# OnurBasci/Real_Time_Path_Tracing_With_SpatioTemporal_Filtering

Measured on AMD Instinct MI355X. Metric: Mray/s (closest-hit queries / whole-frame time: G-buffer + gradient + trace + a-trous), higher is better.
Workload: dtype f32

## Files before the change

include/rtpt.h:

```cpp
#ifndef RTPT_H
#define RTPT_H

#include <stddef.h>
#include <stdint.h>

#ifdef __cplusplus
extern "C" {
#endif

#define RTPT_ABI_VERSION 5

#define RTPT_OK 0
#define RTPT_E_INVALID (-1)
#define RTPT_E_NOMEM (-2)
#define RTPT_E_DEVICE (-3)
#define RTPT_E_NO_SCENE (-4)
#define RTPT_E_NO_GPU (-5)


typedef struct rtpt_push_constants {
  uint32_t sample_batch;
  uint32_t frameNumber;
  uint32_t _pad0[2];
  float cameraPos[3];
// ... 161 lines not shown
struct rtpt_scene_build_info {
  uint32_t builder, fallback;
  uint32_t n_primitives;
  uint32_t n_nodes, depth;
  uint32_t leaf_pairs;
  float build_ms;
  float upload_ms;
};
int rtpt_scene_build_info(rtpt_ctx* ctx, struct rtpt_scene_build_info* out);
int rtpt_scene_rebuild(rtpt_ctx* ctx);

int rtpt_scene_set_instances(rtpt_ctx* ctx, const float* instance_xforms, uint32_t n_instances);

int rtpt_debug_upload_info(rtpt_ctx* ctx, uint64_t out[4]);

int rtpt_debug_live_device_bytes(uint64_t* out);

int rtpt_debug_reuse_info(rtpt_ctx* ctx, uint64_t out[4]);

int rtpt_debug_reproj_info(rtpt_ctx* ctx, uint64_t out[4]);

int rtpt_debug_defer_info(rtpt_ctx* ctx, uint64_t out[4]);


int rtpt_gbuffer(rtpt_ctx* ctx, const rtpt_ubo* ubo, uint32_t y0, uint32_t y1);
int rtpt_temporal_gradient(rtpt_ctx* ctx, const rtpt_push_constants* pc, uint32_t y0, uint32_t y1);
int rtpt_raytrace(rtpt_ctx* ctx, const rtpt_push_constants* pc, uint32_t y0, uint32_t y1);
int rtpt_temporal_filter(rtpt_ctx* ctx, const rtpt_push_constants* pc, const rtpt_ubo* ubo,
                         uint32_t y0, uint32_t y1);
int rtpt_end_frame(rtpt_ctx* ctx);

int rtpt_present(rtpt_ctx* ctx, void* dst_device, uint32_t y0, uint32_t y1);
int rtpt_present_target(rtpt_ctx* ctx, void* dst_device, uint32_t y0, uint32_t y1);

int rtpt_modulate(rtpt_ctx* ctx, uint32_t y0, uint32_t y1);

int rtpt_sync(rtpt_ctx* ctx);
int rtpt_readback(rtpt_ctx* ctx, rtpt_plane which, void* dst, size_t bytes);
int rtpt_set_plane(rtpt_ctx* ctx, rtpt_plane which, const void* src, size_t bytes);
int rtpt_reset_counters(rtpt_ctx* ctx);
int rtpt_set_count_rows(rtpt_ctx* ctx, uint32_t y0, uint32_t y1);
#define RTPT_DEBUG_HIT_ID 0x1u
#define RTPT_DEBUG_PREV_PIXEL 0x2u
int rtpt_enable_debug(rtpt_ctx* ctx, uint32_t mask);

typedef enum rtpt_kernel_id {
// ... 66 lines not shown
```

real_time_path_tracing_with_spatiotemporal_filtering_amd/abi.py:

```python
from __future__ import annotations

import ctypes as C
import os

import numpy as np

PKG_DIR = os.path.dirname(os.path.abspath(__file__))
REPO_DIR = os.path.dirname(PKG_DIR)
LIB_PATH = os.environ.get("RTPT_LIB_PATH") or os.path.join(PKG_DIR, "librtpt_hip.so")
HEADER_PATH = os.path.join(REPO_DIR, "include", "rtpt.h")

RTPT_OK, RTPT_E_INVALID, RTPT_E_NOMEM, RTPT_E_DEVICE, RTPT_E_NO_SCENE, RTPT_E_NO_GPU = 0, -1, -2, -3, -4, -5
FLAG_EXACT_FILTER, FLAG_FORCE_BVH, FLAG_DIRECT_FILTER, FLAG_NO_PATH_COMPACTION = 0x1, 0x2, 0x4, 0x8
FLAG_EXT_ADAPTIVE_ALPHA, FLAG_EXT_GAUSS5, FLAG_EXT_POW2_STRIDE, FLAG_EXT_DISOCCLUSION = 0x10, 0x20, 0x40, 0x80
FLAG_EXT_VARIANCE = 0x100
FLAG_SINGLE_LAUNCH_PATHS = 0x200
FLAG_NO_FILTER_FUSION = 0x400
FLAG_EXT_SVGF_VARIANCE = 0x800
FLAG_EXT_MASK = 0x9F0
FLAG_DEVICE_BVH_BUILD = 0x1000
FLAG_DEVICE_BVH_SAH = 0x2000
FLAG_EXT_DEMODULATE = 0x8000
FLAG_DEVICE_FLATTEN = 0x4000
BVH_BUILDER_HOST_SAH, BVH_BUILDER_DEVICE_LBVH = 0, 1
# ... 80 lines not shown
        ("max_segments", C.c_uint32), ("samples_per_pixel", C.c_uint32),
        ("sigma_n", C.c_int32), ("sigma_z", C.c_float), ("sigma_l", C.c_float), ("alpha", C.c_float),
        ("light_radius", C.c_float), ("light_intensity", C.c_float), ("first_hit_light_divisor", C.c_float),
        ("fov_slope", C.c_float), ("pixel_jitter", C.c_float), ("ray_offset", C.c_float), ("ray_tmax", C.c_float),
        ("flags", C.c_uint32), ("device", C.c_int32),
    ]


assert C.sizeof(PushConstants) == 112 and C.sizeof(Ubo) == 384 and C.sizeof(SceneBuildInfo) == 32

SYMBOLS = [
    "rtpt_config_default", "rtpt_create", "rtpt_destroy", "rtpt_resize", "rtpt_last_error", "rtpt_set_stream", "rtpt_bind_plane",
    "rtpt_plane_ptr", "rtpt_plane_bytes", "rtpt_set_external_history", "rtpt_stream_wait", "rtpt_scene_upload", "rtpt_gbuffer", "rtpt_temporal_gradient",
    "rtpt_raytrace", "rtpt_temporal_filter", "rtpt_end_frame", "rtpt_sync", "rtpt_readback", "rtpt_set_plane",
    "rtpt_reset_counters", "rtpt_set_count_rows", "rtpt_enable_debug", "rtpt_timing_enable", "rtpt_timing_collect", "rtpt_kernel_name",
    "rtpt_selftest_math", "rtpt_selftest_exhaustive", "rtpt_selftest_div", "rtpt_selftest_trace", "rtpt_util_look_at", "rtpt_util_perspective", "rtpt_util_load_obj", "rtpt_util_bvh_check", "rtpt_util_bvh_check_pairs",
    "rtpt_scene_set_materials", "rtpt_util_load_obj_materials", "rtpt_util_bvh_refit_check", "rtpt_set_external_guides",
    "rtpt_present", "rtpt_debug_bvh_check", "rtpt_present_target", "rtpt_scene_build_info", "rtpt_scene_rebuild",
    "rtpt_debug_reuse_info", "rtpt_debug_bvh_topology", "rtpt_scene_set_instances", "rtpt_debug_upload_info",
    "rtpt_debug_live_device_bytes", "rtpt_modulate", "rtpt_debug_reproj_info", "rtpt_debug_defer_info",
    "rtpt_scene_set_textures", "rtpt_selftest_texture", "rtpt_util_load_obj_texcoords", "rtpt_util_load_obj_map_kd",
    "rtpt_selftest_texture_lod", "rtpt_selftest_texture_footprint", "rtpt_util_texture_chain", "rtpt_selftest_contract",
    "rtpt_scene_set_materials_ext", "rtpt_util_load_obj_materials_ext", "rtpt_selftest_bounce",
    "rtpt_util_load_obj_materials_ni", "rtpt_selftest_refract",
]

CONTRACT_WORDS = ((6, 1), (6, 3), (3, 1), (3, 3), (2, 1), (1, 1), (2, 2), (4, 1), (1, 3), (1, 2), (1, 1), (1, 1), (19, 4), (2, 1),
                  (3, 2), (9, 1), (12, 3), (13, 3), (12, 3), (36, 2), (10, 1), (3, 3), (3, 6))

_lib = None


def load() -> C.CDLL:
    global _lib
    if _lib is not None:
        return _lib
    if not os.path.exists(LIB_PATH):
        raise RtptLibraryMissing(
            f"{LIB_PATH} not found: build it with `python -c 'import __graft_entry__ as g; g.build()'` "
            "(hipcc --offload-arch=gfx950).  There is no CPU fallback for the hot path.")
    lib = C.CDLL(LIB_PATH)
    vp, u32, sz = C.c_void_p, C.c_uint32, C.c_size_t
    lib.rtpt_last_error.restype = C.c_char_p
    lib.rtpt_last_error.argtypes = [vp]
    lib.rtpt_kernel_name.restype = C.c_char_p
    lib.rtpt_kernel_name.argtypes = [C.c_int]
    sigs = {
# ... 22 lines not shown
        "rtpt_set_plane": [vp, C.c_int, vp, sz],
        "rtpt_reset_counters": [vp],
        "rtpt_enable_debug": [vp, u32],
        "rtpt_set_count_rows": [vp, u32, u32],
        "rtpt_timing_enable": [vp, C.c_int],
        "rtpt_timing_collect": [vp, C.POINTER(C.c_double * K_COUNT), C.POINTER(u32 * K_COUNT)],
        "rtpt_selftest_math": [vp, C.c_int, vp, vp, sz],
        "rtpt_selftest_exhaustive": [vp, C.c_int, vp, vp],
        "rtpt_selftest_div": [vp, C.c_int, C.c_uint32, C.c_uint32, vp, vp],
        "rtpt_selftest_trace": [vp, vp, sz, vp, vp],
        "rtpt_selftest_contract": [vp, C.c_int, vp, vp, sz],
        "rtpt_util_load_obj": [C.c_char_p, vp, C.POINTER(u32), vp, C.POINTER(u32)],
        "rtpt_util_bvh_check": [vp, u32, C.POINTER(C.c_uint64 * 8)],
        "rtpt_util_bvh_check_pairs": [vp, u32, C.c_int, C.POINTER(C.c_uint64 * 8)],
        "rtpt_scene_set_materials": [vp, vp, u32, vp, u32],
        "rtpt_util_bvh_refit_check": [vp, vp, u32, C.POINTER(C.c_uint64 * 8)],
        "rtpt_debug_bvh_check": [vp, C.POINTER(C.c_uint64 * 8)],
        "rtpt_scene_build_info": [vp, C.POINTER(SceneBuildInfo)],
        "rtpt_scene_rebuild": [vp],
        "rtpt_debug_bvh_topology": [vp, vp, C.POINTER(u32), vp, C.POINTER(u32)],
        "rtpt_debug_reuse_info": [vp, C.POINTER(C.c_uint64 * 4)],
        "rtpt_debug_reproj_info": [vp, C.POINTER(C.c_uint64 * 4)],
        "rtpt_debug_defer_info": [vp, C.POINTER(C.c_uint64 * 4)],
        "rtpt_scene_set_instances": [vp, vp, u32],
        "rtpt_debug_upload_info": [vp, C.POINTER(C.c_uint64 * 4)],
        "rtpt_debug_live_device_bytes": [C.POINTER(C.c_uint64)],
        "rtpt_util_load_obj_materials": [C.c_char_p, vp, C.POINTER(u32), vp, C.POINTER(u32)],
        "rtpt_scene_set_textures": [vp, vp, vp, u32, vp, u32, vp, sz],
        "rtpt_selftest_texture": [vp, u32, vp, sz, vp],
        "rtpt_util_load_obj_texcoords": [C.c_char_p, vp, C.POINTER(u32)],
        "rtpt_util_load_obj_map_kd": [C.c_char_p, vp, C.POINTER(sz), C.POINTER(u32)],
        "rtpt_selftest_texture_lod": [vp, u32, vp, vp, sz, vp],
        "rtpt_selftest_texture_footprint": [vp, vp, sz, u32, vp, vp],
        "rtpt_util_texture_chain": [u32, u32, C.POINTER(u32), C.POINTER(C.c_uint64)],
        "rtpt_scene_set_materials_ext": [vp, vp, u32, vp, u32],
        "rtpt_util_load_obj_materials_ext": [C.c_char_p, vp, C.POINTER(u32), vp, C.POINTER(u32)],
        "rtpt_selftest_bounce": [vp, vp, vp, sz],
        "rtpt_util_load_obj_materials_ni": [C.c_char_p, vp, C.POINTER(u32), vp, C.POINTER(u32)],
        "rtpt_selftest_refract": [vp, vp, vp, sz],
    }
    for name, args in sigs.items():
        fn = getattr(lib, name)
        fn.restype = C.c_int
        fn.argtypes = args
    lib.rtpt_util_look_at.restype = None
    lib.rtpt_util_look_at.argtypes = [vp, vp, vp, vp]
# ... 198 lines not shown
    def scene_build_info(self) -> dict:
        info = SceneBuildInfo()
        _check(self._lib.rtpt_scene_build_info(self._h, C.byref(info)))
        return {name: getattr(info, name) for name, _ in SceneBuildInfo._fields_}

    def scene_rebuild(self):
        _check(self._lib.rtpt_scene_rebuild(self._h))

    def reuse_info(self) -> dict:
        out = (C.c_uint64 * 4)()
        _check(self._lib.rtpt_debug_reuse_info(self._h, C.byref(out)))
        return dict(zip(("frames_skipped", "reproj_stores", "reproj_loads", "tags_invalidated"), (int(v) for v in out)))

    def reproj_info(self) -> dict:
        out = (C.c_uint64 * 4)()
        _check(self._lib.rtpt_debug_reproj_info(self._h, C.byref(out)))
        return dict(zip(("stores", "loads", "invalidations", "plane_bytes"), (int(v) for v in out)))

    def defer_info(self) -> dict:
        out = (C.c_uint64 * 4)()
        _check(self._lib.rtpt_debug_defer_info(self._h, C.byref(out)))
        return dict(zip(("recorded", "launched_in_trace", "launched_alone", "spare_bytes"), (int(v) for v in out)))

    def set_materials(self, tri_material: np.ndarray | None, materials: np.ndarray | None):
        if tri_material is None or materials is None:
            _check(self._lib.rtpt_scene_set_materials(self._h, None, 0, None, 0))
            return
        tri = np.ascontiguousarray(tri_material, np.uint32)
        mats = np.ascontiguousarray(materials, np.float32).reshape(-1, 6)
        _check(self._lib.rtpt_scene_set_materials(self._h, _ptr(tri), len(tri), _ptr(mats), len(mats)))

    def set_textures(self, tri_uv=None, tri_texture=None, textures=None, texels=None):
        if tri_uv is None or tri_texture is None or textures is None or texels is None:
            _check(self._lib.rtpt_scene_set_textures(self._h, None, None, 0, None, 0, None, 0))
            return
        uv = np.ascontiguousarray(tri_uv, np.float32).reshape(-1, 6)
        tri = np.ascontiguousarray(tri_texture, np.uint32).ravel()
        if len(uv) != len(tri):
            raise ValueError("one uv record and one texture index per triangle")
        desc = np.ascontiguousarray(textures, np.uint32).reshape(-1, 4)
        tex = np.ascontiguousarray(texels, np.float32).reshape(-1, 4)
        _check(self._lib.rtpt_scene_set_textures(self._h, _ptr(uv), _ptr(tri), len(tri), _ptr(desc), len(desc), _ptr(tex), len(tex)))

    def gbuffer(self, ubo: Ubo, y0=0, y1=0):
        _check(self._lib.rtpt_gbuffer(self._h, C.byref(ubo), y0, y1))

# ... 167 lines not shown
```

real_time_path_tracing_with_spatiotemporal_filtering_amd/csrc/api_context.hip:

```cpp
#include "api_internal.hpp"

#include <atomic>

namespace rtpt_impl {

thread_local std::string g_err;

int fail(int code, const std::string& msg) {
  g_err = msg;
  return code;
}


size_t frame_blocks(const rtpt_ctx* c) {
  const size_t tiles = ((static_cast<size_t>(c->cfg.width) + 63) / 64) * ((static_cast<size_t>(c->cfg.row_end - c->cfg.row_begin) + 3) / 4);
  return std::max(tiles, static_cast<size_t>(c->n_cu > 0 ? c->n_cu : 256) * 8);
}
int ensure_stack_spill(rtpt_ctx* c, size_t blocks) {
  if (!c->scene.use_bvh) return RTPT_OK;
  const size_t depth = static_cast<size_t>(c->scene.tree.bvh_depth + 2 < 8 ? 8 : c->scene.tree.bvh_depth + 2);
  const size_t lds = std::min<size_t>(depth, static_cast<size_t>(c->bvh_stack_lds));
  if (depth <= lds || blocks <= c->stack_spill_blocks) return RTPT_OK;
  if (c->stack_spill.ptr) {
    hipError_t e = hipStreamSynchronize(c->stream);
// ... 329 lines not shown
  if (const char* v = std::getenv("RTPT_LBVH_ORDER")) c->lbvh_by_height = !std::strcmp(v, "height");
  if (const char* v = std::getenv("RTPT_NO_TRACE_FUSION")) c->fuse_trace = std::atoi(v) == 0;
  if (const char* v = std::getenv("RTPT_NO_FRAME_REUSE")) c->frame_reuse = std::atoi(v) == 0;
  if (const char* v = std::getenv("RTPT_NO_REPROJ_REUSE")) c->reproj_reuse = std::atoi(v) == 0;
  if (const char* v = std::getenv("RTPT_TRACE_POOL")) c->trace_pool = std::atoi(v) != 0;
  if (const char* v = std::getenv("RTPT_TEX_BOUNCE_SPREAD")) {
    const float f = std::strtof(v, nullptr);
    if (f > 0.0f && f <= 64.0f) c->tex_bounce_spread = f;
  }
  if (const char* v = std::getenv("RTPT_PT_WINDOW")) c->trace_window = static_cast<uint32_t>(std::max(0, std::atoi(v)));
  if (const char* v = std::getenv("RTPT_CHAIN_G1")) c->filter_policy.chain_g_pin = std::atoi(v);
  if (const char* v = std::getenv("RTPT_CHAIN_GENERIC")) c->filter_policy.chain_generic = std::atoi(v);
  if (const char* v = std::getenv("RTPT_CHAIN_WG_PER_CU")) c->filter_policy.chain_wg_per_cu = std::atoi(v);
  if (const char* v = std::getenv("RTPT_CHAIN_SKEW")) {
    c->filter_policy.chain_skew = c->filter_policy.chain_skew2 = std::atoi(v);
    if (const char* comma = std::strchr(v, ',')) c->filter_policy.chain_skew2 = std::atoi(comma + 1);
  }
  if (const char* v = std::getenv("RTPT_CHAIN_BW")) c->filter_policy.chain_bw = std::atoi(v);
  if (const char* v = std::getenv("RTPT_NO_FINAL_DEFER")) c->final_defer = std::atoi(v) == 0;
  if (const char* v = std::getenv("RTPT_FINAL_FRONT")) {
    c->filter_policy.final_front = std::atoi(v);
    if (const char* comma = std::strchr(v, ',')) c->filter_policy.final_front_share = std::atoi(comma + 1);
  }
  if (const char* v = std::getenv("RTPT_CHAIN_SW")) c->filter_policy.chain_sw = std::atoi(v);
  if (const char* v = std::getenv("RTPT_CHAIN_SW_G1")) c->filter_policy.chain_sw_g1 = std::atoi(v);
  if (const char* v = std::getenv("RTPT_CHAIN_SW_G3")) c->filter_policy.chain_sw_g3 = std::atoi(v);
  if (const char* v = std::getenv("RTPT_CHAIN_MAX")) c->chain_max = std::max(1, std::min(3, std::atoi(v)));
  if (const char* v = std::getenv("RTPT_CHAIN_FINAL")) c->chain_final = std::atoi(v) != 0;
  if (const char* v = std::getenv("RTPT_BVH_STACK_LDS")) c->bvh_stack_lds = std::max(1, std::atoi(v));
  if (const char* v = std::getenv("RTPT_CHAIN_MIN_PIXELS")) c->chain_min_pixels = std::atoll(v);
  int rc = alloc_planes(c);
  if (rc != RTPT_OK) {
    rtpt_destroy(c);
    return rc;
  }
  *out = c;
  return RTPT_OK;
}

int rtpt_destroy(rtpt_ctx* c) {
  if (!c) return RTPT_OK;
  (void)hipSetDevice(c->device);
  (void)final_flush(c);
  if (c->own_stream) (void)hipStreamSynchronize(c->own_stream);
  for (auto& t : c->timed) {
    (void)hipEventDestroy(t.start);
// ... 145 lines not shown
  }
  if (mask != c->debug_mask) reuse_invalidate(c, nullptr);
  c->debug_mask = mask;
  return RTPT_OK;
}

int rtpt_debug_reuse_info(rtpt_ctx* c, uint64_t out[4]) {
  if (!c || !out) return fail(RTPT_E_INVALID, "NULL argument");
  for (int i = 0; i < 4; i++) out[i] = c->reuse_info[i];
  return RTPT_OK;
}

int rtpt_debug_reproj_info(rtpt_ctx* c, uint64_t out[4]) {
  if (!c || !out) return fail(RTPT_E_INVALID, "NULL argument");
  for (int i = 0; i < 3; i++) out[i] = c->reproj_info[i];
  out[3] = c->reproj.bytes;
  return RTPT_OK;
}

int rtpt_debug_defer_info(rtpt_ctx* c, uint64_t out[4]) {
  if (!c || !out) return fail(RTPT_E_INVALID, "NULL argument");
  for (int i = 0; i < 3; i++) out[i] = c->defer_info[i];
  out[3] = c->color[3].bytes;
  return RTPT_OK;
}

int rtpt_debug_live_device_bytes(uint64_t* out) {
  if (!out) return fail(RTPT_E_INVALID, "NULL argument");
  *out = g_live_device_bytes.load();
  return RTPT_OK;
}

int rtpt_debug_upload_info(rtpt_ctx* c, uint64_t out[4]) {
  if (!c || !out) return fail(RTPT_E_INVALID, "NULL argument");
  for (int i = 0; i < 4; i++) out[i] = c->upload_info[i];
  return RTPT_OK;
}

int rtpt_sync(rtpt_ctx* c) {
  if (!c) return fail(RTPT_E_INVALID, "ctx is NULL");
  HIP_TRY(hipSetDevice(c->device));
  FLUSH_FILTER(c);
  HIP_TRY(hipStreamSynchronize(c->stream));
  return RTPT_OK;
}

// ... 113 lines not shown
```

real_time_path_tracing_with_spatiotemporal_filtering_amd/csrc/api_internal.hpp:

```cpp
#pragma once
#include <hip/hip_runtime.h>

#include <algorithm>
#include <cmath>
#include <cstdio>
#include <cstdlib>
#include <cfloat>
#include <cstring>
#include <new>
#include <string>
#include <vector>

#include "../../include/rtpt.h"
#include "bvh.hpp"
#include "kernels.hpp"
#include "rtpt_math.hpp"


namespace rtpt_impl {


extern thread_local std::string g_err;
int fail(int code, const std::string& msg);

// ... 203 lines not shown
  rt::GbufferArgs pending_gb{};
  bool pending_gb_valid = false;
  bool fuse_trace = true;
  bool frame_reuse = true;
  uint64_t scene_gen = 0;
  K1Key pending_key;
  PlaneTag<K0Key> tag_vis[2], tag_worldpos, tag_depth, tag_normals;
  PlaneTag<K1Key> tag_gradient;
  uint64_t reuse_info[4] = {0, 0, 0, 0};
  bool reproj_reuse = true;
  Buf reproj;
  PlaneTag<ReprojKey> tag_reproj;
  PlaneTag<ReprojKey> reproj_last;
  uint64_t reproj_info[4] = {0, 0, 0, 0};
  bool trace_pool = false;
  uint32_t trace_window = 0;
  float tex_bounce_spread = rt::kTexBounceSpread;
  Buf path_pool;
  rt::FilterPolicy filter_policy;
  bool final_defer = true;
  bool deferred_valid = false;
  DeferredFinal deferred;
  uint64_t defer_info[4] = {0, 0, 0, 0};
  std::vector<FilterCall> pending;
  int chain_max = 2;
  bool chain_final = false;
  int64_t chain_min_pixels = 1000000;

  int bvh_stack_lds = 16;
  Buf stack_spill;
  size_t stack_spill_blocks = 0;

  int timing_period = 0;
  uint64_t frames_ended = 0;
  bool timing_now() const { return timing_period > 0 && (frames_ended % static_cast<uint64_t>(timing_period)) == 0; }
  std::vector<TimedLaunch> timed;
  std::vector<hipEvent_t> event_pool;

  uint32_t rows() const { return cfg.row_end - cfg.row_begin; }
  Rows stored_rows() const { return Rows(cfg.row_begin, cfg.row_end); }
  bool width_fits_i16() const { return cfg.width < 30000 && cfg.height < 30000; }
  size_t pixels() const { return static_cast<size_t>(rows()) * cfg.width; }
};

namespace rtpt_impl {

// ... 64 lines not shown
```

real_time_path_tracing_with_spatiotemporal_filtering_amd/csrc/api_passes.hip:

```cpp
#include "api_internal.hpp"

namespace rtpt_impl {
void reuse_invalidate(rtpt_ctx* c, const Buf* b) {
  auto kill = [&](auto& tag, const Buf* of) {
    if ((!b || b == of) && tag.valid) {
      tag.valid = false;
      c->reuse_info[3]++;
    }
  };
  kill(c->tag_vis[0], &c->vis[0]);
  kill(c->tag_vis[1], &c->vis[1]);
  kill(c->tag_worldpos, &c->worldpos);
  kill(c->tag_depth, &c->depth);
  kill(c->tag_normals, &c->normals);
  kill(c->tag_gradient, &c->gradient);
  const bool lut = b == &c->scene.lut[0] || b == &c->scene.lut[1];
  if (lut) kill(c->tag_gradient, b);
  if (!b || lut || b == &c->worldpos || b == &c->vis[0] || b == &c->vis[1]) {
    if (c->tag_reproj.valid) c->reproj_info[2]++;
    c->tag_reproj.valid = false;
    c->reproj_last.valid = false;
  }
}
}
// ... 367 lines not shown
  if (take) {
    FrameState& fr = c->frame;
    if (!c->color[fr.color_spare].ptr) {
      if ((rc = alloc_buf(c->color[fr.color_spare], c->pixels() * 16))) return rc;
      HIP_TRY(hipMemsetAsync(c->color[fr.color_spare].ptr, 0, c->pixels() * 16, c->stream));
    }
    std::swap(fr.color_of_role[ROLE_IMAGE], fr.color_spare);
  }
  a.image = static_cast<float4*>(c->color[c->frame.color_of_role[ROLE_IMAGE]].ptr);
  c->frame.alpha_depth[c->frame.color_of_role[ROLE_IMAGE]] = true;
  if ((rc = ensure_stack_spill(c, std::max<size_t>(frame_blocks(c), rt::pathtrace_grid_blocks(a, fused ? &c->pending_gb : nullptr))))) return rc;
  a.scene = scene_view(c);
  if (joined) {
    c->pending_gb.scene = a.scene;
    c->pending_gb_valid = false;
    if (reused)
      c->reuse_info[0]++;
    else
      tag_outputs(c, c->pending_gb, &c->pending_key);
  }
  {
    Timer tm(c, joined ? RTPT_K_GBUFFER_PATHTRACE : RTPT_K_PATHTRACE);
    rt::launch_pathtrace(a, fused ? &c->pending_gb : nullptr, tex_view(c), c->scene.materials_specular, c->stream,
                         take ? &c->deferred.args : nullptr, &c->filter_policy);
  }
  if (take) {
    c->deferred_valid = false;
    c->defer_info[1]++;
  }
  return launch_check(fused ? "gbuffer + temporal_gradient + raytrace" : "raytrace");
}

}

namespace {

bool is_final(int k, int max_it) { return k == max_it && (k & 1); }

struct Reach {
  int stride;
  int64_t reach;
};
Reach filter_reach(uint32_t ext, int k) {
  const int stride = (ext & rt::kExtPow2Stride) ? (1 << (k - 1)) : k;
  return {stride, static_cast<int64_t>(stride) * ((ext & rt::kExtGauss5) ? 2 : 1)};
}
Rows rows_read(const rtpt_ctx* c, uint32_t y0, uint32_t y1, int64_t reach) {
// ... 413 lines not shown
```

real_time_path_tracing_with_spatiotemporal_filtering_amd/csrc/final_split.hpp:

```cpp
#pragma once
#include <cstdint>

#if defined(__HIPCC__)
#define RTPT_FS_HD __host__ __device__
#else
#define RTPT_FS_HD
#endif

namespace rt {

struct FinalSplit {
  uint32_t n_front, n_tail;
  uint32_t front_items, items;
  uint32_t tiles_x, n_tiles;
};

enum : uint32_t { kFinalRoleTile = 0, kFinalRoleFront = 1, kFinalRoleTail = 2 };
struct FinalRole {
  uint32_t role;
  uint32_t index;
};

RTPT_FS_HD inline FinalRole final_role(const FinalSplit& sp, uint32_t block) {
  const uint32_t t = block - sp.n_front;
  if (t < sp.n_tiles) return FinalRole{kFinalRoleTile, t};
  if (block < sp.n_front) return FinalRole{kFinalRoleFront, block};
  return FinalRole{kFinalRoleTail, t - sp.n_tiles};
}
RTPT_FS_HD inline uint32_t final_grid(const FinalSplit& sp) { return sp.n_front + sp.n_tiles + sp.n_tail; }

constexpr uint32_t kFinalWholeListItems = 32;
inline FinalSplit final_split_plan(uint32_t items, uint32_t tiles_x, uint32_t tiles_y, uint32_t n_cu, uint32_t per_cu, int front, int share) {
  const uint32_t cu8 = (n_cu + 7u) / 8u;
  auto clamp = [](int v, uint32_t hi) { return v < 0 ? 0u : (static_cast<uint32_t>(v) > hi ? hi : static_cast<uint32_t>(v)); };
  const uint32_t front_max = cu8 * (per_cu - 1u);
  uint32_t front_slots = front <= 0 ? 0u : (static_cast<uint32_t>(front) < per_cu ? cu8 * static_cast<uint32_t>(front) : static_cast<uint32_t>(front) / 8u);
  front_slots = front_slots < front_max ? front_slots : front_max;
  FinalSplit sp;
  sp.tiles_x = tiles_x;
  sp.n_tiles = tiles_x * tiles_y;
  sp.items = items;
  if (share < 0) share = items >= kFinalWholeListItems * 8u * front_slots ? 100 : 75;
  sp.front_items = front_slots ? static_cast<uint32_t>(static_cast<uint64_t>(items) * clamp(share, 100u) / 100u) : 0u;
  auto group = [](uint32_t n_items, uint32_t slots_per_xcd) {
    const uint32_t per_xcd = (n_items + 7u) / 8u;
    return n_items ? 8u * (per_xcd < slots_per_xcd ? per_xcd : slots_per_xcd) : 0u;
  };
  sp.n_front = group(sp.front_items, front_slots);
  sp.n_tail = group(items - sp.front_items, cu8 * per_cu - front_slots);
  return sp;
}

}
```

real_time_path_tracing_with_spatiotemporal_filtering_amd/csrc/kernels.hip:

```cpp
#include <cstdlib>

#include "atrous_comb.hpp"
#include "final_split.hpp"
#include "pathtrace_tile.hpp"
#include "select.hpp"

namespace rt {
namespace {

__global__ void k_scene_prepare(ScenePrepArgs a) {
  uint32_t i = blockIdx.x * blockDim.x + threadIdx.x;
  if (i >= a.n_tris) return;
  {
    const float* t = a.tris + 9 * static_cast<size_t>(i);
    f3 v0 = ld3(t), v1 = ld3(t + 3), v2 = ld3(t + 6);
    f3 e1 = v1 - v0, e2 = v2 - v0;
    f3 nn = exact::cross(e1, e2);
    a.isect_id[3 * i] = make_float4(v0.x, v0.y, v0.z, e1.x);
    a.isect_id[3 * i + 1] = make_float4(e1.y, e1.z, e2.x, e2.y);
    a.isect_id[3 * i + 2] = make_float4(e2.z, nn.x, nn.y, nn.z);
    f3 n = exact::normalize(nn);
    a.shade[3 * i] = make_float4(v0.x, v0.y, v0.z, n.x);
    a.shade[3 * i + 1] = make_float4(v1.x, v1.y, v1.z, n.y);
    a.shade[3 * i + 2] = make_float4(v2.x, v2.y, v2.z, n.z);
// ... 97 lines not shown
}

template <int BVH, bool DEMOD, int TEX, int SPEC>
__global__ __launch_bounds__(kPtThreads)
__attribute__((amdgpu_waves_per_eu(kPtBvhWaves, kPtBvhWaves)))
void k_gbuffer_pathtrace(PathtraceArgs a, GbufferArgs g, TexView tex) {
  gbuffer_pathtrace_body<BVH, DEMOD, TEX, SPEC>(a, g, tex);
}
template <bool DEMOD, int TEX, int SPEC>
__global__ __launch_bounds__(kPtThreads)
__attribute__((amdgpu_waves_per_eu(kPtWaves, kPtWaves)))
void k_gbuffer_pathtrace_small(PathtraceArgs a, GbufferArgs g, TexView tex) {
  gbuffer_pathtrace_body<0, DEMOD, TEX, SPEC>(a, g, tex);
}

template <int CW>
__global__ __launch_bounds__(kPtThreads)
__attribute__((amdgpu_waves_per_eu(kPtWaves, kPtWaves)))
void k_pathtrace_final(PathtraceArgs a, TexView tex, AtrousArgs f, FinalSplit sp) {
  static_assert(kPtThreads == kShThreads && kPtRows == kShWaves, "the two bodies share the workgroup shape");
  const FinalRole r = final_role(sp, blockIdx.x);
  if (r.role == kFinalRoleTile) {
    pathtrace_tile<0, true, false, false, 0, 0, 1>(a, tex, r.index, sp.tiles_x, a.tiles_y);
  } else {
    extern __shared__ __attribute__((aligned(16))) unsigned char final_lds[];
    const bool front = r.role == kFinalRoleFront;
#if RTPT_TILE_TIMELINE
    FilterTimelineScope tl_(r.role, front ? r.index : sp.n_front + r.index);
#endif
    comb_items<CW, true, false, false, 1, false, false, true, true>(f, final_lds, r.index, front ? sp.n_front : sp.n_tail,
                                                                       front ? 0u : sp.front_items, front ? sp.front_items : sp.items);
  }
}

template <int BVH, int TEX, int SPEC>
__global__ __launch_bounds__(kPtThreads) void k_pathtrace_queue(PathtraceArgs a, TexView tex) {
  extern __shared__ __attribute__((aligned(16))) uint32_t stack[];
  PathState& st = *reinterpret_cast<PathState*>(stack);
  __shared__ uint32_t wave_cnt[kPtRows];
  __shared__ uint32_t q_base;
  __shared__ unsigned int block_rays;
  const int tid = threadIdx.y * kBlockX + threadIdx.x;
  const int wave = __builtin_amdgcn_readfirstlane(static_cast<int>(threadIdx.y));
  const uint32_t lane = threadIdx.x;
  if (tid == 0) block_rays = 0;
  const f3 light_c = ld3(a.light_c);
// ... 112 lines not shown
bool pathtrace_uses_pool(const PathtraceArgs& a) {
  return a.pool_slab && a.scene.use_bvh && a.scene.leaf_pairs && a.compact && a.spp == 1;
}
size_t pathtrace_pool_bytes(int W, int rows) {
  return static_cast<size_t>((W + kBlockX - 1) / kBlockX) * ((rows + kPoolRows - 1) / kPoolRows) * (7u * kPoolPaths * sizeof(float4));
}
#else
constexpr int kPoolRows = kPtRows;
bool pathtrace_uses_pool(const PathtraceArgs&) { return false; }
size_t pathtrace_pool_bytes(int, int) { return 0; }
#endif
bool pathtrace_takes_final(const PathtraceArgs& a, const TexView& tex, int specular) {
  return !a.scene.use_bvh && a.compact && a.spp == 1 && !a.albedo && !tex.records && !specular && !pathtrace_uses_pool(a) && a.g.y1 > a.g.y0;
}
uint32_t pathtrace_grid_blocks(const PathtraceArgs& a, const GbufferArgs* gb) {
  const uint32_t gx = (a.g.W + kBlockX - 1) / kBlockX;
  const int tr = pathtrace_uses_pool(a) ? kPoolRows : kPtRows;
  return gx * ((a.g.y1 - a.g.y0 + tr - 1) / tr + (gb ? (gb->g.y1 - gb->g.y0 + kBlockY - 1) / kBlockY : 0));
}
static FinalSplit final_split(const PathtraceArgs& a, const AtrousArgs& f, const FilterPolicy& pol, uint32_t tiles_x, uint32_t tiles_y) {
  const uint32_t n_cu = a.n_cu > 0 ? static_cast<uint32_t>(a.n_cu) : 256u;
  const uint32_t per_cu = static_cast<uint32_t>(kPtWaves * 4 / kShWaves);
  const uint32_t items = static_cast<uint32_t>(f.tiles_x) * static_cast<uint32_t>(f.tiles_y) * static_cast<uint32_t>(f.stride);
  return final_split_plan(items, tiles_x, tiles_y, n_cu, per_cu, pol.final_front, pol.final_front_share);
}
void launch_pathtrace(const PathtraceArgs& a, const GbufferArgs* gb, const TexView& tex, int specular, hipStream_t s, const AtrousArgs* fin,
                      const FilterPolicy* pol) {
  if (a.g.y1 <= a.g.y0) return;
  dim3 block(kBlockX, kPtRows);
  const bool pool = pathtrace_uses_pool(a);
  const int tile_rows = pool ? kPoolRows : kPtRows;
  const uint32_t tiles_y = (a.g.y1 - a.g.y0 + tile_rows - 1) / tile_rows;
  const dim3 grid((a.g.W + kBlockX - 1) / kBlockX, tiles_y + (gb ? (gb->g.y1 - gb->g.y0 + kBlockY - 1) / kBlockY : 0), 1);
  const size_t stack_bytes = a.scene.use_bvh ? static_cast<size_t>(a.scene.stack_lds) * kPtThreads * 4 : 0;
  size_t dyn = stack_bytes > sizeof(PathState) ? stack_bytes : sizeof(PathState);
  if (fin) {
    if (gb || !pol || !fin->reproj_in || !pathtrace_takes_final(a, tex, specular)) std::abort();
    dyn = dyn > final_role_lds(*fin) ? dyn : final_role_lds(*fin);
  }
  PathtraceArgs b = a;
  b.tiles_y = tiles_y;
  b.multi_off = static_cast<uint32_t>(dyn / 4);
  const size_t dyn_queue = dyn;
  if (a.spp > 1) dyn += 4 * kPtThreads * 4;
  const uint32_t phase0 = a.first_window ? a.first_window : pt_first_window(a.scene.use_bvh != 0);
  const bool split = a.spp == 1 && a.compact && a.queue[0] && a.queue_count && a.max_segments > phase0 &&
                     (a.max_segments <= 2 * phase0 || a.queue[1]);
  b.seg_begin = 0;
  b.seg_end = split ? phase0 : a.max_segments;
  b.q_in = nullptr;
  b.q_in_count = nullptr;
  b.q_out = split ? a.queue[0] : nullptr;
  b.q_out_count = split ? a.queue_count : nullptr;
  if (split) (void)hipMemsetAsync(a.queue_count, 0, 2 * kPathQueues * sizeof(uint32_t), s);
  if (fin) {
    const FinalSplit sp = final_split(a, *fin, *pol, grid.x, tiles_y);
    const dim3 grid1(final_grid(sp));
    hipLaunchKernelGGL(k_pathtrace_final<kFinalRoleCw>, grid1, block, dyn, s, b, tex, *fin, sp);
  } else
#if RTPT_AB_VARIANTS
  if (pool) {
    if (gb)
      hipLaunchKernelGGL((k_pathtrace_pool<true>), grid, block, dyn, s, b, *gb);
    else
      hipLaunchKernelGGL((k_pathtrace_pool<false>), grid, block, dyn, s, b, GbufferArgs{});
  } else
#endif
  with_mode3(scene_mode(a.scene), [&](auto mode) {
    constexpr int M = decltype(mode)::value;
    with_bool(a.albedo != nullptr, [&](auto demod) {
      constexpr bool D = decltype(demod)::value;
      with_mode3(tex_mode(tex), [&](auto tmode) {
        constexpr int T = decltype(tmode)::value;
        with_mode3(spec_mode(specular), [&](auto spec) {
          constexpr int S = decltype(spec)::value;
          if (gb) {
            if constexpr (M != 0)
              hipLaunchKernelGGL((k_gbuffer_pathtrace<M, D, T, S>), grid, block, dyn, s, b, *gb, tex);
            else
              hipLaunchKernelGGL((k_gbuffer_pathtrace_small<D, T, S>), grid, block, dyn, s, b, *gb, tex);
// ... 42 lines not shown
```

real_time_path_tracing_with_spatiotemporal_filtering_amd/csrc/kernels.hpp:

```cpp
#pragma once

#include <hip/hip_runtime.h>
#include <stdint.h>

#include "bvh.hpp"
#include "texture.hpp"

namespace rt {

struct SceneView {
  const float4* isect_id;
  const float4* isect_leaf;
  const uint32_t* leaf_ids;
  const float4* shade;
  const BvhNodeQ* nodes;
  const float* bvh_grid;
  uint32_t n_tris;
  uint32_t use_bvh;
  uint32_t paired;
  uint32_t leaf_pairs;
  uint32_t stack_depth;
  uint32_t stack_lds;
  uint32_t* stack_spill;
  const float4* materials;
// ... 219 lines not shown
void launch_fan_pairs(uint32_t n_pairs, const float* tris, uint32_t* all_paired, hipStream_t s);
constexpr uint32_t kLbvhMaxLevels = 128;
constexpr uint32_t kLbvhHeaderWords = 2 + kLbvhMaxLevels;
struct LbvhArgs {
  uint32_t n_prims;
  uint32_t prim_w;
  const float* tris;
  BvhNodeQ* nodes;
  uint32_t* leaf_order;
  uint32_t* refit_order;
  uint32_t* header;
  uint32_t by_height;
};
size_t lbvh_scratch_bytes(uint32_t n_prims, bool by_height);
hipError_t launch_lbvh_build(const LbvhArgs& a, void* scratch, size_t scratch_bytes, hipStream_t s);
size_t sah_scratch_bytes(uint32_t n_prims);
hipError_t launch_sah_build(const LbvhArgs& a, void* scratch, size_t scratch_bytes, hipStream_t s);
void launch_lut(const LutArgs& a, hipStream_t s);
void launch_gbuffer(const GbufferArgs& a, hipStream_t s);
void launch_ray_tables(int W, int H, float p00, float p11, float* dvx, float* dvy, hipStream_t s);
void launch_gradient(const GradientArgs& a, hipStream_t s);
struct FilterPolicy;
void launch_pathtrace(const PathtraceArgs& a, const GbufferArgs* gb, const TexView& tex, int specular, hipStream_t s, const AtrousArgs* fin = nullptr,
                      const FilterPolicy* pol = nullptr);
bool pathtrace_takes_final(const PathtraceArgs& a, const TexView& tex, int specular);
bool pathtrace_fuses_gbuffer(const PathtraceArgs& a, const GbufferArgs& g);
uint32_t pathtrace_grid_blocks(const PathtraceArgs& a, const GbufferArgs* gb);
bool pathtrace_uses_pool(const PathtraceArgs& a);
size_t pathtrace_pool_bytes(int W, int rows);
void launch_atrous(const AtrousArgs& a, bool final_pass, hipStream_t s);
bool atrous_final_fuses_present(const AtrousArgs& a);
bool atrous_final_plain_comb(const AtrousArgs& a);
bool atrous_final_role(AtrousArgs& a);
struct FilterPolicy {
  int chain_g_pin = 0;
  int chain_generic = 0;
  int chain_wg_per_cu = 0;
  int chain_sw = 0;
  int chain_sw_g1 = 0, chain_sw_g3 = 0;
  int chain_skew = -1, chain_skew2 = -1;
  int chain_bw = 0;
  int final_front = 1, final_front_share = -1;
};
void launch_atrous_chain(const AtrousArgs& a, int levels, bool final_pass, const FilterPolicy& pol, hipStream_t s);
bool atrous_chain_supported(int k0, int levels, uint32_t n_tris);
hipError_t prepare_device_atrous_chain();
hipError_t prepare_device_atrous();
void launch_stamp_depth(const FrameGeom& g, float4* color, const float* depth, hipStream_t s);
void launch_present(const FrameGeom& g, const float4* image, const float4* albedo, uint32_t* dst, hipStream_t s);
void launch_modulate(const FrameGeom& g, const float4* image, const float4* albedo, float4* shaded, hipStream_t s);
void launch_selftest_math(int op, const float* in, float* out, size_t n, hipStream_t s);
void launch_selftest_exhaustive(int op, unsigned long long* out, hipStream_t s);
void launch_selftest_div(int mode, uint32_t pass, unsigned long long* out, hipStream_t s);
void launch_selftest_trace(const SceneView& scene, const float* rays, size_t n, float tmax, uint32_t* out_id,
                           float* out_t, hipStream_t s);
constexpr int kContractFns = 23;
constexpr uint32_t kContractWords[kContractFns][2] = {
    {6, 1},  {6, 3},  {3, 1},  {3, 3},  {2, 1},  {1, 1},  {2, 2},  {4, 1},  {1, 3},  {1, 2},  {1, 1},  {1, 1},
    {19, 4}, {2, 1},  {3, 2},  {9, 1},  {12, 3}, {13, 3}, {12, 3}, {36, 2}, {10, 1}, {3, 3},  {3, 6}};
void launch_selftest_contract(int fn, const uint32_t* in, uint32_t* out, size_t n, hipStream_t s);
void launch_selftest_bounce(const float* in, float* out, size_t n, hipStream_t s);
void launch_selftest_refract(const float* in, float* out, size_t n, hipStream_t s);
void launch_selftest_texture(const TexDesc* desc, const float4* texels, const float* uv, size_t n, float4* out, hipStream_t s);
void launch_selftest_texture_lod(const TexDesc* desc, const uint32_t* lv, const float4* texels, const float* uv, const float* lod, size_t n,
                                 float4* out, hipStream_t s);
// ... 5 lines not shown
```

real_time_path_tracing_with_spatiotemporal_filtering_amd/csrc/pathtrace_tile.hpp:

```cpp
#pragma once

#include "gbuffer_tile.hpp"
#include "shade_segment.hpp"

namespace rt {
namespace {

constexpr int kPtRows = 4;
constexpr int kPtThreads = kBlockX * kPtRows;

__device__ __forceinline__ void enqueue_paths(const PathtraceArgs& a, uint32_t region, uint32_t* wave_cnt, uint32_t* bcast,
                                              bool alive, int wave, uint32_t lane, uint32_t pixg, uint32_t rng, f3 o, f3 d, f3 acc) {
  const unsigned long long m = __ballot(alive);
  if (lane == 0) wave_cnt[wave] = static_cast<uint32_t>(__builtin_popcountll(m));
  __syncthreads();
  uint32_t before = 0, total = 0;
#pragma unroll
  for (int w = 0; w < kPtRows; w++) {
    const uint32_t c = wave_cnt[w];
    if (w < wave) before += c;
    total += c;
  }
  if (wave == 0 && lane == 0) *bcast = total ? atomicAdd(a.q_out_count + region, total) : 0u;
  __syncthreads();
// ... 167 lines not shown
    }
    if (a.seg_end < a.max_segments) {
      const uint32_t pixg = (static_cast<uint32_t>(tile_y0 + static_cast<int>(pix >> 6)) << 16) |
                            static_cast<uint32_t>(tile_x0 + static_cast<int>(pix & 63u));
      const uint32_t blk = tile_lin<ROLE>(role_lin);
      enqueue_paths(a, blk % kPathQueues, wave_cnt, &q_base, alive, wave, lane, pixg, rng, o, d, acc);
    }
  }
  __syncthreads();
  if (a.spp > 1) {
    const int x = tile_x0 + static_cast<int>(lane), y = tile_y0 + wave;
    if (x < a.g.W && y < a.g.y1) {
      const float ns = static_cast<float>(a.spp);
      const size_t gi = static_cast<size_t>(y - a.g.row_base) * a.g.W + x;
      if (GB)
        store_rgb(a.image + gi, f3{sum_r[tid] / ns, sum_g[tid] / ns, sum_b[tid] / ns});
      else
        a.image[gi] = make_float4(sum_r[tid] / ns, sum_g[tid] / ns, sum_b[tid] / ns, a.depth[gi]);
    }
  }
  add_block_rays(a, rays, &block_rays, tid, tile_lin<ROLE>(role_lin));
}

template <int BVH, bool DEMOD, int TEX, int SPEC>
__device__ __forceinline__ void gbuffer_pathtrace_body(const PathtraceArgs& a, const GbufferArgs& g, const TexView& tex) {
  if (blockIdx.y < a.tiles_y) {
    pathtrace_tile<BVH, true, true, DEMOD, TEX, SPEC>(a, tex);
  } else {
    extern __shared__ __attribute__((aligned(16))) uint32_t stack[];
#if RTPT_TILE_TIMELINE
    TimelineScope tl_(0, (blockIdx.y - a.tiles_y) * gridDim.x + blockIdx.x);
#endif
    gbuffer_tile<BVH>(g, blockIdx.x, blockIdx.y - a.tiles_y, stack, a.image, a.g.y0, a.g.y1);
  }
}

constexpr int kPtBvhWaves = 8;

}
}
```

Measured before the change: 32050.

## Batch empty screen columns into multi-tile runs in the fused final pathtrace kernel

Finds tile columns whose screen footprint overlaps no triangle bounds and assigns them to 'run' workgroups. Each run workgroup shades several vertically stacked tiles with a light or sky lookup only, instead of launching one full pathtrace tile per tile. This reduces workgroup count and per-tile overhead for empty regions. In exchange it adds a host-side scan over triangle bounds for every launch and a new grid role. Debug counters are exposed through a new API.

```diff
diff --git a/include/rtpt.h b/include/rtpt.h
--- a/include/rtpt.h
+++ b/include/rtpt.h
@@ -207,6 +207,8 @@
 
 int rtpt_debug_defer_info(rtpt_ctx* ctx, uint64_t out[4]);
 
+int rtpt_debug_empty_run_info(rtpt_ctx* ctx, uint64_t out[4]);
+
 
 int rtpt_gbuffer(rtpt_ctx* ctx, const rtpt_ubo* ubo, uint32_t y0, uint32_t y1);
 int rtpt_temporal_gradient(rtpt_ctx* ctx, const rtpt_push_constants* pc, uint32_t y0, uint32_t y1);
diff --git a/real_time_path_tracing_with_spatiotemporal_filtering_amd/abi.py b/real_time_path_tracing_with_spatiotemporal_filtering_amd/abi.py
--- a/real_time_path_tracing_with_spatiotemporal_filtering_amd/abi.py
+++ b/real_time_path_tracing_with_spatiotemporal_filtering_amd/abi.py
@@ -126,7 +126,7 @@
     "rtpt_scene_set_textures", "rtpt_selftest_texture", "rtpt_util_load_obj_texcoords", "rtpt_util_load_obj_map_kd",
     "rtpt_selftest_texture_lod", "rtpt_selftest_texture_footprint", "rtpt_util_texture_chain", "rtpt_selftest_contract",
     "rtpt_scene_set_materials_ext", "rtpt_util_load_obj_materials_ext", "rtpt_selftest_bounce",
-    "rtpt_util_load_obj_materials_ni", "rtpt_selftest_refract",
+    "rtpt_util_load_obj_materials_ni", "rtpt_selftest_refract", "rtpt_debug_empty_run_info",
 ]
 
 CONTRACT_WORDS = ((6, 1), (6, 3), (3, 1), (3, 3), (2, 1), (1, 1), (2, 2), (4, 1), (1, 3), (1, 2), (1, 1), (1, 1), (19, 4), (2, 1),
@@ -195,6 +195,7 @@
         "rtpt_debug_reuse_info": [vp, C.POINTER(C.c_uint64 * 4)],
         "rtpt_debug_reproj_info": [vp, C.POINTER(C.c_uint64 * 4)],
         "rtpt_debug_defer_info": [vp, C.POINTER(C.c_uint64 * 4)],
+        "rtpt_debug_empty_run_info": [vp, C.POINTER(C.c_uint64 * 4)],
         "rtpt_scene_set_instances": [vp, vp, u32],
         "rtpt_debug_upload_info": [vp, C.POINTER(C.c_uint64 * 4)],
         "rtpt_debug_live_device_bytes": [C.POINTER(C.c_uint64)],
@@ -439,6 +440,11 @@
         _check(self._lib.rtpt_debug_defer_info(self._h, C.byref(out)))
         return dict(zip(("recorded", "launched_in_trace", "launched_alone", "spare_bytes"), (int(v) for v in out)))
 
+    def empty_run_info(self) -> dict:
+        out = (C.c_uint64 * 4)()
+        _check(self._lib.rtpt_debug_empty_run_info(self._h, C.byref(out)))
+        return dict(zip(("full_columns", "run_workgroups", "run_tiles", "run_len"), (int(v) for v in out)))
+
     def set_materials(self, tri_material: np.ndarray | None, materials: np.ndarray | None):
         if tri_material is None or materials is None:
             _check(self._lib.rtpt_scene_set_materials(self._h, None, 0, None, 0))
diff --git a/real_time_path_tracing_with_spatiotemporal_filtering_amd/csrc/api_context.hip b/real_time_path_tracing_with_spatiotemporal_filtering_amd/csrc/api_context.hip
--- a/real_time_path_tracing_with_spatiotemporal_filtering_amd/csrc/api_context.hip
+++ b/real_time_path_tracing_with_spatiotemporal_filtering_amd/csrc/api_context.hip
@@ -375,6 +375,7 @@
     c->filter_policy.final_front = std::atoi(v);
     if (const char* comma = std::strchr(v, ',')) c->filter_policy.final_front_share = std::atoi(comma + 1);
   }
+  if (const char* v = std::getenv("RTPT_EMPTY_RUN")) c->filter_policy.empty_run = std::max(0, std::atoi(v));
   if (const char* v = std::getenv("RTPT_CHAIN_SW")) c->filter_policy.chain_sw = std::atoi(v);
   if (const char* v = std::getenv("RTPT_CHAIN_SW_G1")) c->filter_policy.chain_sw_g1 = std::atoi(v);
   if (const char* v = std::getenv("RTPT_CHAIN_SW_G3")) c->filter_policy.chain_sw_g3 = std::atoi(v);
@@ -566,6 +567,13 @@
   if (!c || !out) return fail(RTPT_E_INVALID, "NULL argument");
   for (int i = 0; i < 3; i++) out[i] = c->defer_info[i];
   out[3] = c->color[3].bytes;
+  return RTPT_OK;
+}
+
+int rtpt_debug_empty_run_info(rtpt_ctx* c, uint64_t out[4]) {
+  if (!c || !out) return fail(RTPT_E_INVALID, "NULL argument");
+  for (int i = 0; i < 3; i++) out[i] = c->empty_run_info[i];
+  out[3] = static_cast<uint64_t>(c->filter_policy.empty_run);
   return RTPT_OK;
 }
 
diff --git a/real_time_path_tracing_with_spatiotemporal_filtering_amd/csrc/api_internal.hpp b/real_time_path_tracing_with_spatiotemporal_filtering_amd/csrc/api_internal.hpp
--- a/real_time_path_tracing_with_spatiotemporal_filtering_amd/csrc/api_internal.hpp
+++ b/real_time_path_tracing_with_spatiotemporal_filtering_amd/csrc/api_internal.hpp
@@ -249,6 +249,7 @@
   bool deferred_valid = false;
   DeferredFinal deferred;
   uint64_t defer_info[4] = {0, 0, 0, 0};
+  uint32_t empty_run_info[3] = {0, 0, 0};
   std::vector<FilterCall> pending;
   int chain_max = 2;
   bool chain_final = false;
diff --git a/real_time_path_tracing_with_spatiotemporal_filtering_amd/csrc/api_passes.hip b/real_time_path_tracing_with_spatiotemporal_filtering_amd/csrc/api_passes.hip
--- a/real_time_path_tracing_with_spatiotemporal_filtering_amd/csrc/api_passes.hip
+++ b/real_time_path_tracing_with_spatiotemporal_filtering_amd/csrc/api_passes.hip
@@ -413,7 +413,7 @@
   {
     Timer tm(c, joined ? RTPT_K_GBUFFER_PATHTRACE : RTPT_K_PATHTRACE);
     rt::launch_pathtrace(a, fused ? &c->pending_gb : nullptr, tex_view(c), c->scene.materials_specular, c->stream,
-                         take ? &c->deferred.args : nullptr, &c->filter_policy);
+                         take ? &c->deferred.args : nullptr, &c->filter_policy, c->empty_run_info);
   }
   if (take) {
     c->deferred_valid = false;
diff --git a/real_time_path_tracing_with_spatiotemporal_filtering_amd/csrc/final_split.hpp b/real_time_path_tracing_with_spatiotemporal_filtering_amd/csrc/final_split.hpp
--- a/real_time_path_tracing_with_spatiotemporal_filtering_amd/csrc/final_split.hpp
+++ b/real_time_path_tracing_with_spatiotemporal_filtering_amd/csrc/final_split.hpp
@@ -13,9 +13,11 @@
   uint32_t n_front, n_tail;
   uint32_t front_items, items;
   uint32_t tiles_x, n_tiles;
+  uint32_t n_runs, run_len;
+  uint32_t runs_per_col, tiles_y;
 };
 
-enum : uint32_t { kFinalRoleTile = 0, kFinalRoleFront = 1, kFinalRoleTail = 2 };
+enum : uint32_t { kFinalRoleTile = 0, kFinalRoleFront = 1, kFinalRoleTail = 2, kFinalRoleRun = 3 };
 struct FinalRole {
   uint32_t role;
   uint32_t index;
@@ -25,9 +27,39 @@
   const uint32_t t = block - sp.n_front;
   if (t < sp.n_tiles) return FinalRole{kFinalRoleTile, t};
   if (block < sp.n_front) return FinalRole{kFinalRoleFront, block};
-  return FinalRole{kFinalRoleTail, t - sp.n_tiles};
+  const uint32_t u = t - sp.n_tiles;
+  if (u < sp.n_runs) return FinalRole{kFinalRoleRun, u};
+  return FinalRole{kFinalRoleTail, u - sp.n_runs};
 }
-RTPT_FS_HD inline uint32_t final_grid(const FinalSplit& sp) { return sp.n_front + sp.n_tiles + sp.n_tail; }
+RTPT_FS_HD inline uint32_t final_grid(const FinalSplit& sp) { return sp.n_front + sp.n_tiles + sp.n_runs + sp.n_tail; }
+
+RTPT_FS_HD inline uint32_t tile_order_column(uint32_t tiles_x, uint32_t col) {
+  return (col & 1u) ? (tiles_x - 1u) / 2u + (col + 1u) / 2u : (tiles_x - 1u) / 2u - col / 2u;
+}
+
+struct FinalRun {
+  uint32_t column, row0, rows;
+};
+RTPT_FS_HD inline FinalRun final_run(const FinalSplit& sp, uint32_t index) {
+  const uint32_t c = index / sp.runs_per_col, row0 = (index - c * sp.runs_per_col) * sp.run_len;
+  const uint32_t left = sp.tiles_y - row0;
+  return FinalRun{tile_order_column(sp.tiles_x, sp.n_tiles / sp.tiles_y + c), row0, left < sp.run_len ? left : sp.run_len};
+}
+
+constexpr int kTileColumnPixels = 64;
+template <class Bounds>
+inline uint32_t final_full_columns(const Bounds* bounds, uint32_t n, int W, int y0, int y1, uint32_t tiles_x) {
+  for (uint32_t col = tiles_x; col > 0; col--) {
+    const int cx0 = static_cast<int>(tile_order_column(tiles_x, col - 1u)) * kTileColumnPixels;
+    const int cx1 = (cx0 + kTileColumnPixels < W ? cx0 + kTileColumnPixels : W) - 1;
+    for (uint32_t i = 0; i < n; i++) {
+      const Bounds& b = bounds[i];
+      if (b.x0 > b.x1) continue;
+      if (!(b.x0 > cx1 || b.x1 < cx0 || b.y0 > y1 - 1 || b.y1 < y0)) return col;
+    }
+  }
+  return 0u;
+}
 
 constexpr uint32_t kFinalWholeListItems = 32;
 inline FinalSplit final_split_plan(uint32_t items, uint32_t tiles_x, uint32_t tiles_y, uint32_t n_cu, uint32_t per_cu, int front, int share) {
@@ -48,6 +80,20 @@
   };
   sp.n_front = group(sp.front_items, front_slots);
   sp.n_tail = group(items - sp.front_items, cu8 * per_cu - front_slots);
+  sp.n_runs = sp.run_len = sp.runs_per_col = sp.tiles_y = 0u;
+  return sp;
+}
+
+inline FinalSplit final_split_plan(uint32_t items, uint32_t tiles_x, uint32_t tiles_y, uint32_t n_cu, uint32_t per_cu, int front, int share,
+                                   uint32_t full_cols, uint32_t run_len) {
+  FinalSplit sp = final_split_plan(items, tiles_x, tiles_y, n_cu, per_cu, front, share);
+  if (run_len == 0u || full_cols >= tiles_x || tiles_y == 0u) return sp;
+  run_len = run_len < tiles_y ? run_len : tiles_y;
+  sp.n_tiles = full_cols * tiles_y;
+  sp.run_len = run_len;
+  sp.runs_per_col = (tiles_y + run_len - 1u) / run_len;
+  sp.tiles_y = tiles_y;
+  sp.n_runs = (tiles_x - full_cols) * sp.runs_per_col;
   return sp;
 }
 
diff --git a/real_time_path_tracing_with_spatiotemporal_filtering_amd/csrc/kernels.hip b/real_time_path_tracing_with_spatiotemporal_filtering_amd/csrc/kernels.hip
--- a/real_time_path_tracing_with_spatiotemporal_filtering_amd/csrc/kernels.hip
+++ b/real_time_path_tracing_with_spatiotemporal_filtering_amd/csrc/kernels.hip
@@ -143,6 +143,13 @@
   const FinalRole r = final_role(sp, blockIdx.x);
   if (r.role == kFinalRoleTile) {
     pathtrace_tile<0, true, false, false, 0, 0, 1>(a, tex, r.index, sp.tiles_x, a.tiles_y);
+  } else if (r.role == kFinalRoleRun) {
+    extern __shared__ __attribute__((aligned(16))) unsigned char final_lds[];
+#if RTPT_TILE_TIMELINE
+    FilterTimelineScope tl_(r.role, sp.n_front + sp.n_tail + r.index);
+#endif
+    const FinalRun run = final_run(sp, r.index);
+    pathtrace_empty_run(a, run.column, run.row0, run.rows, sp.n_tiles + r.index, reinterpret_cast<unsigned int*>(final_lds));
   } else {
     extern __shared__ __attribute__((aligned(16))) unsigned char final_lds[];
     const bool front = r.role == kFinalRoleFront;
@@ -301,10 +308,18 @@
   const uint32_t n_cu = a.n_cu > 0 ? static_cast<uint32_t>(a.n_cu) : 256u;
   const uint32_t per_cu = static_cast<uint32_t>(kPtWaves * 4 / kShWaves);
   const uint32_t items = static_cast<uint32_t>(f.tiles_x) * static_cast<uint32_t>(f.tiles_y) * static_cast<uint32_t>(f.stride);
-  return final_split_plan(items, tiles_x, tiles_y, n_cu, per_cu, pol.final_front, pol.final_front_share);
+  static_assert(kTileColumnPixels == kBlockX, "final_full_columns and the tile kernel agree on a column");
+  const bool runs = pol.empty_run > 0 && a.cull && a.max_segments > 0;
+  const uint32_t full_cols = runs ? final_full_columns(a.bounds, a.scene.n_tris, a.g.W, a.g.y0, a.g.y1, tiles_x) : tiles_x;
+  return final_split_plan(items, tiles_x, tiles_y, n_cu, per_cu, pol.final_front, pol.final_front_share, full_cols,
+                          runs ? static_cast<uint32_t>(pol.empty_run) : 0u);
 }
 void launch_pathtrace(const PathtraceArgs& a, const GbufferArgs* gb, const TexView& tex, int specular, hipStream_t s, const AtrousArgs* fin,
-                      const FilterPolicy* pol) {
+                      const FilterPolicy* pol, uint32_t* run_info) {
+  if (run_info) {
+    run_info[0] = a.g.y1 > a.g.y0 ? static_cast<uint32_t>((a.g.W + kBlockX - 1) / kBlockX) : 0u;
+    run_info[1] = run_info[2] = 0u;
+  }
   if (a.g.y1 <= a.g.y0) return;
   dim3 block(kBlockX, kPtRows);
   const bool pool = pathtrace_uses_pool(a);
@@ -335,6 +350,11 @@
   if (fin) {
     const FinalSplit sp = final_split(a, *fin, *pol, grid.x, tiles_y);
     const dim3 grid1(final_grid(sp));
+    if (run_info) {
+      run_info[0] = sp.n_runs ? sp.n_tiles / tiles_y : grid.x;
+      run_info[1] = sp.n_runs;
+      run_info[2] = sp.n_runs ? grid.x * tiles_y - sp.n_tiles : 0u;
+    }
     hipLaunchKernelGGL(k_pathtrace_final<kFinalRoleCw>, grid1, block, dyn, s, b, tex, *fin, sp);
   } else
 #if RTPT_AB_VARIANTS
diff --git a/real_time_path_tracing_with_spatiotemporal_filtering_amd/csrc/kernels.hpp b/real_time_path_tracing_with_spatiotemporal_filtering_amd/csrc/kernels.hpp
--- a/real_time_path_tracing_with_spatiotemporal_filtering_amd/csrc/kernels.hpp
+++ b/real_time_path_tracing_with_spatiotemporal_filtering_amd/csrc/kernels.hpp
@@ -265,7 +265,7 @@
 void launch_gradient(const GradientArgs& a, hipStream_t s);
 struct FilterPolicy;
 void launch_pathtrace(const PathtraceArgs& a, const GbufferArgs* gb, const TexView& tex, int specular, hipStream_t s, const AtrousArgs* fin = nullptr,
-                      const FilterPolicy* pol = nullptr);
+                      const FilterPolicy* pol = nullptr, uint32_t* run_info = nullptr);
 bool pathtrace_takes_final(const PathtraceArgs& a, const TexView& tex, int specular);
 bool pathtrace_fuses_gbuffer(const PathtraceArgs& a, const GbufferArgs& g);
 uint32_t pathtrace_grid_blocks(const PathtraceArgs& a, const GbufferArgs* gb);
@@ -275,6 +275,7 @@
 bool atrous_final_fuses_present(const AtrousArgs& a);
 bool atrous_final_plain_comb(const AtrousArgs& a);
 bool atrous_final_role(AtrousArgs& a);
+constexpr int kEmptyRunTiles = 8;
 struct FilterPolicy {
   int chain_g_pin = 0;
   int chain_generic = 0;
@@ -284,6 +285,7 @@
   int chain_skew = -1, chain_skew2 = -1;
   int chain_bw = 0;
   int final_front = 1, final_front_share = -1;
+  int empty_run = kEmptyRunTiles;
 };
 void launch_atrous_chain(const AtrousArgs& a, int levels, bool final_pass, const FilterPolicy& pol, hipStream_t s);
 bool atrous_chain_supported(int k0, int levels, uint32_t n_tris);
diff --git a/real_time_path_tracing_with_spatiotemporal_filtering_amd/csrc/pathtrace_tile.hpp b/real_time_path_tracing_with_spatiotemporal_filtering_amd/csrc/pathtrace_tile.hpp
--- a/real_time_path_tracing_with_spatiotemporal_filtering_amd/csrc/pathtrace_tile.hpp
+++ b/real_time_path_tracing_with_spatiotemporal_filtering_amd/csrc/pathtrace_tile.hpp
@@ -213,6 +213,47 @@
   add_block_rays(a, rays, &block_rays, tid, tile_lin<ROLE>(role_lin));
 }
 
+__device__ __forceinline__ void pathtrace_empty_run(const PathtraceArgs& a, uint32_t bx, uint32_t row0, uint32_t rows, uint32_t slot,
+                                                    unsigned int* block_rays) {
+  const int tid = threadIdx.y * kBlockX + threadIdx.x;
+  const int wave = __builtin_amdgcn_readfirstlane(static_cast<int>(threadIdx.y));
+  if (tid == 0) *block_rays = 0;
+  const float fw = static_cast<float>(a.g.W), fh = static_cast<float>(a.g.H);
+  const f3 light_c = ld3(a.light_c);
+  const int px0 = static_cast<int>(bx) * kBlockX + static_cast<int>(threadIdx.x);
+  unsigned int rays = 0;
+  if (px0 < a.g.W && a.seg_end > 0) {
+    for (uint32_t r = 0; r < rows; r++) {
+      const int py0 = a.g.y0 + static_cast<int>(row0 + r) * kPtRows + wave;
+      if (py0 >= a.g.y1) break;
+      const size_t gi = static_cast<size_t>(py0 - a.g.row_base) * a.g.W + px0;
+      const float depth = a.depth[gi];
+      uint32_t rng = exact::rng_seed(static_cast<uint32_t>(px0), static_cast<uint32_t>(py0), a.frame, a.batch);
+      float u1 = glsl_max(1e-38f, exact::rng_next(rng));
+      float u2 = exact::rng_next(rng);
+      float rad = exact::sqrt_(-2.0f * exact::log_(u1));
+      float sn, cs;
+      exact::sincos2pi(u2, sn, cs);
+      float cx = fmaf_(a.jitter, rad * cs, static_cast<float>(px0) + 0.5f);
+      float cy = fmaf_(a.jitter, rad * sn, static_cast<float>(py0) + 0.5f);
+      float ux = RTPT_DIV_SH(fmaf_(2.0f, cx, -fw), fh);
+      float uy = -RTPT_DIV_SH(fmaf_(2.0f, cy, -fh), fh);
+      const f3 d = exact::normalize(f3{a.slope * ux, a.slope * uy, -1.0f});
+      const f3 o = ld3(a.cam);
+      f3 acc{1.f, 1.f, 1.f};
+      if (py0 >= a.count_y0 && py0 < a.count_y1) rays++;
+      if (a.hit_id) a.hit_id[gi] = 0u;
+      if (ray_hits_light(o, d, light_c, a.light_r2))
+        acc = acc * ld3(a.light_col_first);
+      else
+        acc = acc * sky_color(d);
+      a.image[gi] = make_float4(acc.x, acc.y, acc.z, depth);
+    }
+  }
+  __syncthreads();
+  add_block_rays(a, rays, block_rays, tid, slot);
+}
+
 template <int BVH, bool DEMOD, int TEX, int SPEC>
 __device__ __forceinline__ void gbuffer_pathtrace_body(const PathtraceArgs& a, const GbufferArgs& g, const TexView& tex) {
   if (blockIdx.y < a.tiles_y) {
```

Result: faster. 33070 (median of 6 runs) (+3.2%).
